# aleju/cat-generator

Hardware: AMD Instinct MI355X
Metric: images/sec per G+D step, G32up-c 32x32 RGB bs=128 per GPU (higher is better)
Workload: dtype f32

## Files before the change

### cat-generator_amd/csrc/common.h

```cpp
#pragma once
#include <hip/hip_runtime.h>
#include <algorithm>
#include <stdint.h>
#include <stdio.h>
#include <string.h>
#include "../../include/catgan.h"

namespace cg {

char* err_buf();
int fail(const char* fmt, ...);

inline hipStream_t S(void* s) { return reinterpret_cast<hipStream_t>(s); }

#define CG_HIP(call)                                                              \
    do {                                                                          \
        hipError_t e__ = (call);                                                  \
        if (e__ != hipSuccess)                                                    \
            return cg::fail("%s:%d %s -> %s", __FILE__, __LINE__, #call,          \
                            hipGetErrorString(e__));                              \
    } while (0)

#define CG_LAUNCH_CHECK()                                                         \
    do {                                                                          \
        hipError_t e__ = hipGetLastError();                                       \
        if (e__ != hipSuccess)                                                    \
            return cg::fail("%s:%d kernel launch -> %s", __FILE__, __LINE__,      \
                            hipGetErrorString(e__));                              \
    } while (0)

#define CG_REQUIRE(cond, ...)                                                     \
    do {                                                                          \
        if (!(cond)) return cg::fail(__VA_ARGS__);                                \
    } while (0)

constexpr int kNumCU = 256;

#ifndef CG_TIMING_PROBE
#define CG_TIMING_PROBE 0
#endif
#define CG_PROBE_HALF(fam, T) (((CG_TIMING_PROBE) & (fam)) ? ((T) + 1) / 2 : (T))
constexpr int kEwWgsPerCU = 4, kColReduceWgsPerCU = 1;

enum Opt {
    OPT_SKINNY, OPT_GEMM_BK32, OPT_WINO_BK, OPT_NN_TILE, OPT_TN_TILE, OPT_NN_SPLITS, OPT_TN_SPLITS,
    OPT_XCD_SWIZZLE, OPT_NN_GLDS, OPT_TN_GLDS, OPT_WINO_GLDS, OPT_PAD_SKIP, OPT_WINO3, OPT_COUNT
};
long opt(Opt o);

static inline int cdiv(long a, long b) { return (int)((a + b - 1) / b); }

constexpr size_t kColScratchBytes = 8u << 20;
void* col_scratch(hipStream_t stream);
hipStream_t queue_stream(hipStream_t ref, int cls, int slot);
int queue_class(hipStream_t ref, hipStream_t s);
void wgrad_discard_all();

constexpr int kSkinnyWgradBlocks = 512;
bool skinny_ok(int ngroups, int Cin, int Cout, int kH, int kW, int padH, int padW, int ups);
size_t skinny_wgrad_ws_bytes(int Cin, int Cout);
void skinny_valu_forward(hipStream_t st, const float* x, const float* w, const float* bias, float* y, int N, int H, int W, int Cin, int Cout);
void skinny_valu_wgrad(hipStream_t st, const float* x, const float* dy, float* part, float* bias_part, int N, int H, int W, int Cin, int Cout,
                       int blocks, long ppb);
bool skinny_mfma_ok(int Cin, int Cout, int H, int W);
int skinny_mfma_forward(hipStream_t st, const float* x, const float* w, const float* bias, float* y, int N, int H, int W, int Cin, int Cout);
int skinny_mfma_wgrad(hipStream_t st, const float* x, const float* dy, float* part, float* bias_part, int N, int H, int W, int Cin, int Cout,
                      int max_blocks);

bool head_wgrad_ok(int N, int T, int C, int Co);
int head_wgrad(hipStream_t st, const float* x, const float* dy, float* gw, float* gb, int N, int T, int C, int Co, float scale);
bool wino3_geom_ok(int ngroups, int N, int H, int W, int Cin, int Cout, int kH, int kW, int padH, int padW, int ups);
int wino3_note_pack(hipStream_t st, int n, const float* const* w, float* const* wf, float* const* wb, const int* Cout, const int* Cin,
                    const int* kH, const int* kW, const int* wb_map);
int wino3_forward(hipStream_t st, int ngroups, const float* const* x, const float* const* wpk, const float* const* bias, float* const* y,
                  int N, int H, int W);

static inline int ew_grid(long n, int per_block = 256) {
    long b = (n + per_block - 1) / per_block;
    if (b < 1) b = 1;
    const long cap = (long)kNumCU * kEwWgsPerCU;
    if (b > cap) b = cap;
    return (int)b;
}

__device__ __forceinline__ float u01(uint64_t seed, uint64_t ctr) {
    uint64_t z = seed + (ctr + 1) * 0x9E3779B97F4A7C15ull;
    z = (z ^ (z >> 30)) * 0xBF58476D1CE4E5B9ull;
    z = (z ^ (z >> 27)) * 0x94D049BB133111EBull;
    z = z ^ (z >> 31);
    return (float)(z >> 40) * (1.0f / 16777216.0f);
}
__device__ __forceinline__ float wave_sum(float v) {
#pragma unroll
    for (int off = 32; off > 0; off >>= 1) v += __shfl_down(v, off, 64);
    return v;
}
__device__ __forceinline__ double wave_sum(double v) {
#pragma unroll
    for (int off = 32; off > 0; off >>= 1) v += __shfl_down(v, off, 64);
    return v;
}

#ifndef CG_COL_HANDOVER
#define CG_COL_HANDOVER 3
#endif
__device__ __forceinline__ void st_agent(double* p, double v) {
#if CG_COL_HANDOVER == 4
    const unsigned long long old = __hip_atomic_exchange((unsigned long long*)p, (unsigned long long)__double_as_longlong(v),
                                                         __ATOMIC_RELAXED, __HIP_MEMORY_SCOPE_AGENT);
// ... 98 lines not shown
```

### cat-generator_amd/csrc/gemm.hip

```cpp
#include "common.h"
#include <stdlib.h>
#include <algorithm>
#include <mutex>
#include <type_traits>
#include <unordered_map>
#include <vector>

namespace {

typedef float f32x16 __attribute__((ext_vector_type(16)));
typedef unsigned int u32x4 __attribute__((ext_vector_type(4)));

constexpr int BK = 16;
constexpr unsigned OOB = 0x80000000u;
#ifdef CG_TRACE
__device__ unsigned long long* g_trace;
#define CG_STAMP(slot)                                                                                                  \
    do {                                                                                                                \
        if (threadIdx.x == 0 && g_trace) {                                                                              \
            const long wg = blockIdx.x + (long)gridDim.x * (blockIdx.y + (long)gridDim.y * blockIdx.z);                  \
            g_trace[wg * 8 + (slot)] = wall_clock64();                                                                  \
            if ((slot) == 0) {                                                                                          \
                g_trace[wg * 8 + 4] = __builtin_amdgcn_s_getreg((31 << 11) | 4);                       \
                g_trace[wg * 8 + 5] = __builtin_amdgcn_s_getreg((31 << 11) | 20);                     \
// ... 2189 lines not shown
    Geom g;
    if (check_dims(N, Hp, Wp, Cin, Cout, k, k, pad, pad, 1)) return 1;
    if (geom_phase_dgrad(g, N, Hp, Wp, Cin, Cout, k, pad)) return 1;
    return run_nn(cg::S(stream), g, 1, &dy, &wb_ph, nullptr, &dx_lo, ws, ws_bytes, "cg_conv2d_dgrad_ups2");
}

static size_t wgrad_ws_bytes_groups(int ngroups, int maxg, int N, int Hp, int Wp, int Cin, int Cout, int kH, int kW, int padH, int padW, int ups) {
    Geom g;
    if (ngroups < 1 || ngroups > maxg || conv_geom(g, N, Hp, Wp, Cin, Cout, kH, kW, padH, padW, ups)) return 0;
    const size_t reg = tn_ws_bytes(g, plan_tn(g, ngroups), ngroups);
    return cg::skinny_ok(ngroups, Cin, Cout, kH, kW, padH, padW, ups) ? std::max(reg, cg::skinny_wgrad_ws_bytes(Cin, Cout)) : reg;
}
size_t cg_conv2d_wgrad_workspace_bytes_grouped(int ngroups, int N, int Hp, int Wp, int Cin, int Cout, int kH, int kW,
                                               int padH, int padW, int ups) {
    return wgrad_ws_bytes_groups(ngroups, MAXG, N, Hp, Wp, Cin, Cout, kH, kW, padH, padW, ups);
}
size_t cg_conv2d_wgrad_workspace_bytes_strided(int ngroups, int N, int Hp, int Wp, int Cin, int Cout, int kH, int kW,
                                               int padH, int padW, int ups) {
    return wgrad_ws_bytes_groups(ngroups, kMaxStridedGroups, N, Hp, Wp, Cin, Cout, kH, kW, padH, padW, ups);
}
size_t cg_conv2d_wgrad_workspace_bytes(int N, int Hp, int Wp, int Cin, int Cout, int kH, int kW, int padH, int padW,
                                       int ups) {
    return cg_conv2d_wgrad_workspace_bytes_grouped(1, N, Hp, Wp, Cin, Cout, kH, kW, padH, padW, ups);
}

namespace {
std::mutex g_red_mu;
std::unordered_map<hipStream_t, std::vector<RedJob>> g_red_queue;

long red_cap() { return 0x7fffffffL; }

int small_reduce(hipStream_t st, bool defer, const RedJob& job, int ngroups) {
    if (defer) {
        std::lock_guard<std::mutex> lk(g_red_mu);
        g_red_queue[st].push_back(job);
        g_red_queue[st].back().block0 = ngroups;
        return 0;
    }
    const int nblocks = job.wblocks + job.bblocks;
    const long cap = std::max<long>(1, red_cap() / std::max(1, ngroups));
    dim3 sgrid((unsigned)std::min<long>(nblocks, cap), ngroups);
    if (job.ups)
        hipLaunchKernelGGL(wgrad_reduce_small_kernel<true>, sgrid, dim3(256), 0, st, job.part, job.bias_part, job.rp, job.Cin, job.Cout,
                           job.k, job.KK, job.pad, job.kp, job.S, job.P, job.scale, job.sstride, job.gstride, job.bsstride, job.wblocks, nblocks, 0);
    else
        hipLaunchKernelGGL(wgrad_reduce_small_kernel<false>, sgrid, dim3(256), 0, st, job.part, job.bias_part, job.rp, job.Cin, job.Cout,
                           job.k, job.KK, job.pad, job.kp, job.S, job.P, job.scale, job.sstride, job.gstride, job.bsstride, job.wblocks, nblocks, job.v4);
    CG_LAUNCH_CHECK();
    return 0;
}

int wgrad_impl(void* stream, int ngroups, const float* const* x, const float* const* dy, float* const* gw, float* const* gb, int N,
               int Hp, int Wp, int Cin, int Cout, int kH, int kW, int padH, int padW, int ups, float scale, void* ws, size_t ws_bytes,
               bool defer, long xgs = 0, long dgs = 0, long gws = 0, bool gemm_only = false);
}

int cg_conv2d_wgrad_grouped(void* stream, int ngroups, const float* const* x, const float* const* dy, float* const* gw,
                            float* const* gb, int N, int Hp, int Wp, int Cin, int Cout, int kH, int kW, int padH, int padW,
                            int ups, float scale, void* ws, size_t ws_bytes) {
    return wgrad_impl(stream, ngroups, x, dy, gw, gb, N, Hp, Wp, Cin, Cout, kH, kW, padH, padW, ups, scale, ws, ws_bytes, false);
}

int cg_conv2d_wgrad_grouped_deferred(void* stream, int ngroups, const float* const* x, const float* const* dy, float* const* gw,
                                     float* const* gb, int N, int Hp, int Wp, int Cin, int Cout, int kH, int kW, int padH, int padW,
                                     int ups, float scale, void* ws, size_t ws_bytes) {
    return wgrad_impl(stream, ngroups, x, dy, gw, gb, N, Hp, Wp, Cin, Cout, kH, kW, padH, padW, ups, scale, ws, ws_bytes, true);
}

int cg_conv2d_wgrad_strided(void* stream, int ngroups, const float* x, long x_stride, const float* dy, long dy_stride, float* gw,
                            long gw_stride, int N, int Hp, int Wp, int Cin, int Cout, int kH, int kW, int padH, int padW, int ups,
                            float scale, void* ws, size_t ws_bytes) {
    CG_REQUIRE(x && dy && gw && x_stride > 0 && dy_stride > 0 && gw_stride > 0, "cg_conv2d_wgrad_strided: bad arguments");
    CG_REQUIRE(ngroups >= 1 && ngroups <= kMaxStridedGroups, "cg_conv2d_wgrad_strided: 1..%d groups per launch", kMaxStridedGroups);
    return wgrad_impl(stream, ngroups, &x, &dy, &gw, nullptr, N, Hp, Wp, Cin, Cout, kH, kW, padH, padW, ups, scale, ws, ws_bytes, false,
                      x_stride, dy_stride, gw_stride);
}

int cg_conv2d_wgrad_gemm(void* stream, const float* x, const float* dy, int N, int Hp, int Wp, int Cin, int Cout, int kH, int kW, int padH,
                         int padW, int ups, void* ws, size_t ws_bytes) {
    CG_REQUIRE(x && dy && ws, "cg_conv2d_wgrad_gemm: null pointer");
    CG_REQUIRE(!cg::skinny_ok(1, Cin, Cout, kH, kW, padH, padW, ups), "cg_conv2d_wgrad_gemm: this geometry runs the skinny kernel, not the GEMM");
    float* gw = (float*)ws;
    return wgrad_impl(stream, 1, &x, &dy, &gw, nullptr, N, Hp, Wp, Cin, Cout, kH, kW, padH, padW, ups, 1.f, ws, ws_bytes, false, 0, 0, 0, true);
}

int cg_conv2d_wgrad_pending(void* stream, int* njobs) {
    CG_REQUIRE(njobs, "cg_conv2d_wgrad_pending: null pointer");
    std::lock_guard<std::mutex> lk(g_red_mu);
    auto it = g_red_queue.find(cg::S(stream));
    *njobs = it == g_red_queue.end() ? 0 : (int)it->second.size();
    return 0;
}

int cg_conv2d_wgrad_flush(void* stream) {
    hipStream_t st = cg::S(stream);
    std::vector<RedJob> jobs;
    {
        std::lock_guard<std::mutex> lk(g_red_mu);
        auto it = g_red_queue.find(st);
        if (it == g_red_queue.end() || it->second.empty()) return 0;
        jobs.swap(it->second);
    }
    for (size_t j0 = 0; j0 < jobs.size(); j0 += kRedJobs) {
        RedJobTable t;
        memset(&t, 0, sizeof(t));
        t.n = (int)std::min<size_t>(kRedJobs, jobs.size() - j0);
        int blocks = 0;
        for (int q = 0; q < t.n; ++q) {
            t.j[q] = jobs[j0 + q];
            const int ngroups = t.j[q].block0;
            t.j[q].block0 = blocks;
            blocks += ngroups * (t.j[q].wblocks + t.j[q].bblocks);
        }
        const int wgs = (int)std::min<long>(blocks, red_cap());
        hipLaunchKernelGGL(wgrad_reduce_batch_kernel, dim3(wgs), dim3(256), 0, st, t, blocks);
        CG_LAUNCH_CHECK();
    }
    return 0;
}

namespace {
int wgrad_impl(void* stream, int ngroups, const float* const* x, const float* const* dy, float* const* gw, float* const* gb, int N,
               int Hp, int Wp, int Cin, int Cout, int kH, int kW, int padH, int padW, int ups, float scale, void* ws, size_t ws_bytes,
               bool defer, long xgs, long dgs, long gws_, bool gemm_only) {
    CG_REQUIRE(x && dy && gw, "cg_conv2d_wgrad: null pointer");
    const bool strided = xgs != 0;
    CG_REQUIRE(ngroups >= 1 && ngroups <= (strided ? kMaxStridedGroups : MAXG), "cg_conv2d_wgrad: 1..%d groups per launch", strided ? kMaxStridedGroups : MAXG);
    CG_REQUIRE(!strided || (!gb && !defer), "cg_conv2d_wgrad: strided groups carry no bias gradient and are not deferred");
    TNArgs a;
    memset(&a, 0, sizeof(a));
    if (conv_geom(a.g, N, Hp, Wp, Cin, Cout, kH, kW, padH, padW, ups)) return 1;
    const Geom& g = a.g;
    if (!strided && cg::skinny_ok(ngroups, Cin, Cout, kH, kW, padH, padW, ups) && x[0] && dy[0] && gw[0] && (uintptr_t)x[0] % 16 == 0 && ws &&
        ws_bytes >= cg::skinny_wgrad_ws_bytes(Cin, Cout) && (long)N * Hp * Wp < 0x7fffffffL) {
        hipStream_t st = cg::S(stream);
        const long npix = (long)N * Hp * Wp;
        const long ppb = (npix + cg::kSkinnyWgradBlocks - 1) / cg::kSkinnyWgradBlocks;
        int blocks = (int)((npix + ppb - 1) / ppb);
        float* part = (float*)ws;
        float* bpart = part + (size_t)cg::kSkinnyWgradBlocks * 9 * Cin * Cout;
        float* gb0 = gb ? gb[0] : nullptr;
        if (cg::opt(cg::OPT_SKINNY) == 1 && cg::skinny_mfma_ok(Cin, Cout, Hp, Wp)) {
            blocks = cg::skinny_mfma_wgrad(st, x[0], dy[0], part, gb0 ? bpart : nullptr, N, Hp, Wp, Cin, Cout, cg::kSkinnyWgradBlocks / 2);
            if (blocks < 0) return 1;
        }
        else cg::skinny_valu_wgrad(st, x[0], dy[0], part, gb0 ? bpart : nullptr, N, Hp, Wp, Cin, Cout, blocks, ppb);
        CG_LAUNCH_CHECK();
        RedJob job;
        memset(&job, 0, sizeof(job));
        job.part = part; job.bias_part = bpart;
        job.rp.gw0 = gw[0]; job.rp.gb0 = gb0;
        job.Cin = Cin; job.Cout = Cout; job.k = 3; job.KK = 9; job.pad = 1; job.S = blocks; job.P = 1; job.scale = scale;
        job.sstride = 9L * Cin * Cout; job.gstride = 0; job.bsstride = Cout;
        job.wblocks = cg::cdiv(9L * Cin * Cout, 32); job.bblocks = gb0 ? cg::cdiv(Cout, 32) : 0;
        return small_reduce(st, defer, job, 1);
    }
    if (!strided && !gemm_only && ngroups == 1 && !ups && kH == Hp && kW == Wp && padH == 0 && padW == 0 && cg::opt(cg::OPT_PAD_SKIP) > 0 &&
        cg::opt(cg::OPT_TN_GLDS) && cg::head_wgrad_ok(N, kH * kW, Cin, Cout) && x[0] && dy[0] && gw[0] && (uintptr_t)x[0] % 16 == 0 &&
        (uintptr_t)dy[0] % 16 == 0 && (uintptr_t)gw[0] % 4 == 0)
        return cg::head_wgrad(cg::S(stream), x[0], dy[0], gw[0], gb ? gb[0] : nullptr, N, kH * kW, Cin, Cout, scale) != 0;
    TNPlan p = plan_tn(g, ngroups);
    const size_t need = tn_ws_bytes(g, p, ngroups);
    CG_REQUIRE(ws && ws_bytes >= need, "cg_conv2d_wgrad: workspace too small (%zu < %zu)", ws_bytes, need);
    const int nptr = strided ? 1 : ngroups;
    bool veca = Cin % 4 == 0, vecb = Cout % 4 == 0, any_gb = false;
    for (int i = 0; i < nptr; ++i) {
        CG_REQUIRE(x[i] && dy[i] && gw[i], "cg_conv2d_wgrad: null pointer (group %d)", i);
        veca = veca && ((uintptr_t)x[i] % 16 == 0);
        vecb = vecb && ((uintptr_t)dy[i] % 16 == 0);
        any_gb = any_gb || (gb && gb[i]);
    }
    if (strided) { veca = veca && xgs % 4 == 0; vecb = vecb && dgs % 4 == 0; }
    if (p.pm && !(veca && vecb)) p = plan_tn(g, ngroups, false);
    a.xgs = xgs; a.dgs = dgs;
    set4(a.x0, a.x1, a.x2, a.x3, x, nptr);
    set4(a.d0, a.d1, a.d2, a.d3, dy, nptr);
    a.ngroups = ngroups; a.part = (float*)ws; a.pchunk = p.pchunk;
    a.xcd_swizzle = (int)cg::opt(cg::OPT_XCD_SWIZZLE);
    const int ZP = ngroups * g.nphase;
    const long wplane = (long)g.Ktot * g.Cout;
    a.bias_part = any_gb ? (float*)ws + (size_t)p.splits * ZP * wplane : nullptr;
    hipStream_t st = cg::S(stream);
    dim3 grid(cg::cdiv(g.Ktot, p.tc.bm) * cg::cdiv(g.Cout, p.tc.bn), p.splits, ZP);
    if (p.pm && veca && vecb) a.pm_n = g.M / (g.Hg * g.Wg);
    if (a.pm_n || tng_ok(g, p.pchunk, veca, vecb)) {
        if (p.tc.bm == 128 && p.tc.bn == 128) launch_tng<128, 128, 2, 2>(a, grid, st);
        else if (p.tc.bm == 64 && p.tc.bn == 128) launch_tng<64, 128, 2, 2>(a, grid, st);
        else if (p.tc.bm == 128 && p.tc.bn == 64) launch_tng<128, 64, 2, 2>(a, grid, st);
        else if (p.tc.bm == 64 && p.tc.bn == 64) launch_tng<64, 64, 2, 2>(a, grid, st);
        else launch_tng<128, 32, 4, 1>(a, grid, st);
    }
    else if (p.tc.bm == 128 && p.tc.bn == 128) launch_tn<128, 128, 2, 2>(a, grid, st, veca, vecb);
    else if (p.tc.bm == 64 && p.tc.bn == 128) launch_tn<64, 128, 2, 2>(a, grid, st, veca, vecb);
    else if (p.tc.bm == 128 && p.tc.bn == 64) launch_tn<128, 64, 2, 2>(a, grid, st, veca, vecb);
    else if (p.tc.bm == 64 && p.tc.bn == 64) launch_tn<64, 64, 2, 2>(a, grid, st, veca, vecb);
    else launch_tn<128, 32, 4, 1>(a, grid, st, veca, vecb);
    CG_LAUNCH_CHECK();
    if (gemm_only) return 0;
    const int KK = kH * kW;
    int ci_t = KK == 1 ? 64 : 8;
    while (ci_t > 1 && (size_t)KK * ci_t * 33 * sizeof(float) > 60000) ci_t >>= 1;
    const size_t shb = (size_t)KK * ci_t * 33 * sizeof(float);
    dim3 rgrid(cg::cdiv(Cin, ci_t), cg::cdiv(Cout, 32));
    const long relems = (long)KK * Cin * Cout;
    const long sstride = (long)ZP * wplane;
    const int kp = ups ? phase_kp(kH, padH) : 0;
    if (strided && KK == 1 && !ups && !any_gb && Cin % 32 == 0 && Cout % 32 == 0 && g.nphase == 1) {
        hipLaunchKernelGGL(wgrad_reduce_t_kernel, dim3(Cin / 32, Cout / 32, ngroups), dim3(256), 0, st, (const float*)ws, gw[0], gws_, Cin, Cout,
                           p.splits, sstride, (long)g.nphase * wplane, scale);
        CG_LAUNCH_CHECK();
        return 0;
    }
    if ((long)rgrid.x * rgrid.y < cg::kNumCU) {
        RedJob job;
        memset(&job, 0, sizeof(job));
        job.rp.gws = strided ? gws_ : 0;
        set4(job.rp.gw0, job.rp.gw1, job.rp.gw2, job.rp.gw3, gw, nptr);
        set4(job.rp.gb0, job.rp.gb1, job.rp.gb2, job.rp.gb3, gb, nptr);
        job.part = (const float*)ws; job.bias_part = a.bias_part;
        job.Cin = Cin; job.Cout = Cout; job.k = kH; job.KK = KK; job.pad = padH; job.kp = ups ? kp : 0; job.S = p.splits; job.P = g.nphase;
        job.ups = ups ? 1 : 0; job.scale = scale;
        job.sstride = sstride; job.gstride = (long)g.nphase * wplane; job.bsstride = (long)ZP * Cout;
        job.wblocks = cg::cdiv(relems, 32); job.bblocks = any_gb ? cg::cdiv(Cout, 32) : 0;
        if (defer && KK == 1 && !ups && Cin % 32 == 0 && Cout % 32 == 0 && g.nphase == 1) {
            job.tr = 1; job.wblocks = (Cin / 32) * (Cout / 32);
        } else if (!ups && Cout % 4 == 0 && (uintptr_t)ws % 16 == 0 && sstride % 4 == 0 && job.gstride % 4 == 0) {
            job.v4 = 1; job.wblocks = cg::cdiv(relems, 128);
        }
        return small_reduce(st, defer, job, ngroups);
    }
    for (int gi = 0; gi < ngroups; ++gi) {
        const float* pg = (const float*)ws + (long)gi * g.nphase * wplane;
        float* gwi = strided ? gw[0] + (long)gi * gws_ : gw[gi];
        if (ups)
            hipLaunchKernelGGL(wgrad_reduce_kernel<true>, rgrid, dim3(256), shb, st, pg, gwi, Cin, Cout, kH, KK, padH, kp,
                               p.splits, scale, ci_t, sstride);
        else
            hipLaunchKernelGGL(wgrad_reduce_kernel<false>, rgrid, dim3(256), shb, st, pg, gwi, Cin, Cout, kH, KK, padH,
                               0, p.splits, scale, ci_t, sstride);
        CG_LAUNCH_CHECK();
        if (gb && gb[gi]) {
            hipLaunchKernelGGL(bias_part_reduce_kernel, dim3(cg::cdiv(Cout, 32)), dim3(256), 0, st,
                               (const float*)a.bias_part + (long)gi * g.nphase * Cout, gb[gi], p.splits, g.nphase,
                               (long)ZP * Cout, Cout, scale);
            CG_LAUNCH_CHECK();
        }
    }
    return 0;
}

}
// ... 37 lines not shown
    for (int i0 = 0; i0 < n; i0 += kPackBatch) {
        PackBatch b;
        memset(&b, 0, sizeof(b));
        b.n = std::min(kPackBatch, n - i0);
        int blocks = 0;
        for (int e = 0; e < b.n; ++e) {
            const int i = i0 + e;
            CG_REQUIRE(w_canonical[i] && (wf[i] || wb[i]) && Cout[i] > 0 && Cin[i] > 0 && kH[i] > 0 && kW[i] > 0,
                       "cg_pack_conv_weight_batch: bad layer %d", i);
            b.w[e] = w_canonical[i]; b.wf[e] = wf[i]; b.wb[e] = wb[i];
            b.Cout[e] = Cout[i]; b.Cin[e] = Cin[i]; b.KK[e] = kH[i] * kW[i];
            if (wb_map && wb_map[i]) b.map_mask |= 1ull << e;
            b.first[e] = blocks;
            blocks += cg::cdiv(Cin[i], 32) * cg::cdiv(Cout[i], 32) * b.KK[e];
        }
        b.first[b.n] = blocks;
        hipLaunchKernelGGL(pack_weight_batch_kernel, dim3(blocks), dim3(256), 0, cg::S(stream), b);
        CG_LAUNCH_CHECK();
    }
    return cg::wino3_note_pack(cg::S(stream), n, w_canonical, wf, wb, Cout, Cin, kH, kW, wb_map);
}

size_t cg_pack_conv_weight_ups2_floats(int Cout, int Cin, int k, int pad) {
    if (Cout <= 0 || Cin <= 0 || k <= 0 || (k & 1) == 0 || pad != (k - 1) / 2) return 0;
    const int kp = phase_kp(k, pad);
    return (size_t)4 * kp * kp * Cin * Cout;
}

int cg_pack_conv_weight_ups2(void* stream, const float* w, float* wf_ph, float* wb_ph, int Cout, int Cin, int k, int pad) {
    CG_REQUIRE(w && (wf_ph || wb_ph), "cg_pack_conv_weight_ups2: null pointer");
    CG_REQUIRE(Cout > 0 && Cin > 0 && k > 0 && (k & 1) == 1 && pad == (k - 1) / 2,
               "cg_pack_conv_weight_ups2: needs an odd kernel with pad=(k-1)/2");
    const int kp = phase_kp(k, pad);
    CG_REQUIRE(k * k <= 448, "cg_pack_conv_weight_ups2: kernel too large (%d taps)", k * k);
    const dim3 fgrid(cg::cdiv(Cin, 32), cg::cdiv(Cout, 32));
    if (k == 3 || k == 5) {
        if (k == 3)
            hipLaunchKernelGGL(pack_weight_ups2_fast_kernel<3>, fgrid, dim3(256), 0, cg::S(stream), w, wf_ph, wb_ph, Cout, Cin);
        else
            hipLaunchKernelGGL(pack_weight_ups2_fast_kernel<5>, fgrid, dim3(256), 0, cg::S(stream), w, wf_ph, wb_ph, Cout, Cin);
        CG_LAUNCH_CHECK();
        return 0;
    }
    const int ci_t = pack_ci_tile(Cin, k * k);
    hipLaunchKernelGGL(pack_weight_ups2_kernel, dim3(cg::cdiv(Cin, ci_t), cg::cdiv(Cout, 32)), dim3(256),
                       (size_t)32 * (ci_t * k * k + 1) * sizeof(float), cg::S(stream), w, wf_ph, wb_ph, Cout, Cin, k, pad, kp,
                       ci_t);
    CG_LAUNCH_CHECK();
    return 0;
}

}

void cg::wgrad_discard_all() {
    std::lock_guard<std::mutex> lk(g_red_mu);
    for (auto& kv : g_red_queue) kv.second.clear();
}
```

### cat-generator_amd/csrc/ops.hip

```cpp
#include "common.h"
#include <stdarg.h>
#include <stdlib.h>
#include <algorithm>

namespace cg {
char* err_buf() {
    static thread_local char buf[512] = {0};
    return buf;
}
int fail(const char* fmt, ...) {
    va_list ap;
    va_start(ap, fmt);
    vsnprintf(err_buf(), 512, fmt, ap);
    va_end(ap);
    return 1;
}

namespace {
struct OptDef { const char* name; long dflt; };
const OptDef kOptDefs[OPT_COUNT] = {
    {"CG_SKINNY", 1}, {"CG_GEMM_BK32", 1}, {"CG_WINO_BK", 0}, {"CG_NN_TILE", 0}, {"CG_TN_TILE", 0}, {"CG_NN_SPLITS", 0}, {"CG_TN_SPLITS", 0},
    {"CG_XCD_SWIZZLE", 7}, {"CG_NN_GLDS", 1}, {"CG_TN_GLDS", 1}, {"CG_WINO_GLDS", 1}, {"CG_PAD_SKIP", 20}, {"CG_WINO3", 1},
};
long g_opt_val[OPT_COUNT];
int g_opt_state[OPT_COUNT];
}

}
#include <chrono>
#include <mutex>
#include <unordered_map>
#include <vector>
namespace cg {
void* col_scratch(hipStream_t stream) {
    constexpr int kPool = 8, kReserve = 4;
    static std::unordered_map<hipStream_t, void*> blocks;
    static std::vector<void*> pool;
    static std::mutex mu;
    std::lock_guard<std::mutex> lk(mu);
    auto it = blocks.find(stream);
    if (it != blocks.end()) return it->second;
    hipStreamCaptureStatus st = hipStreamCaptureStatusNone;
    const bool capturing = stream && hipStreamIsCapturing(stream, &st) == hipSuccess && st != hipStreamCaptureStatusNone;
    if (capturing && pool.empty()) {
        cg::fail("column reduce: no scratch block left for a stream first used inside a graph capture (run one pass on it before cg_graph_begin)");
        return nullptr;
    }
    if (!capturing && (int)pool.size() <= kReserve) {
        char* p = nullptr;
        hipStreamCaptureMode mode = hipStreamCaptureModeRelaxed;
        (void)hipThreadExchangeStreamCaptureMode(&mode);
        const bool ok = hipMalloc((void**)&p, kColScratchBytes * kPool) == hipSuccess &&
                        hipMemsetAsync(p, 0, kColScratchBytes * kPool, stream) == hipSuccess &&
                        hipStreamSynchronize(stream) == hipSuccess;
        (void)hipThreadExchangeStreamCaptureMode(&mode);
        if (!ok) {
            (void)hipGetLastError();
            if (pool.empty()) { cg::fail("column reduce: cannot allocate %zu bytes of scratch", kColScratchBytes * kPool); return nullptr; }
        } else
            for (int i = kPool - 1; i >= 0; --i) pool.insert(pool.begin(), p + (size_t)i * kColScratchBytes);
    }
    void* blk = pool.back();
    pool.pop_back();
    blocks[stream] = blk;
    return blk;
}
namespace {
__global__ void queue_probe_spin_k(unsigned long long ticks, int* sink) {
    const unsigned long long t0 = wall_clock64();
    while (wall_clock64() - t0 < ticks) { }
    if (ticks == ~0ull) *sink = 1;
}
struct QueuePool {
    std::vector<hipStream_t> s;
    std::unordered_map<hipStream_t, std::vector<int>> cls;
// ... 1892 lines not shown
```

### cat-generator_amd/csrc/winograd.hip

```cpp
#include "common.h"
#include <algorithm>
#include <type_traits>
#include <stdlib.h>

namespace {

typedef float f32x16 __attribute__((ext_vector_type(16)));

__device__ __forceinline__ float4 ld4(const float* p) { return *reinterpret_cast<const float4*>(p); }
__device__ __forceinline__ float wf4c(const float4& v, int i) { return i == 0 ? v.x : (i == 1 ? v.y : (i == 2 ? v.z : v.w)); }
__device__ __forceinline__ float4 f4add(float4 a, float4 b) { return make_float4(a.x + b.x, a.y + b.y, a.z + b.z, a.w + b.w); }
__device__ __forceinline__ float4 f4sub(float4 a, float4 b) { return make_float4(a.x - b.x, a.y - b.y, a.z - b.z, a.w - b.w); }

template <int MODE>
__global__ __launch_bounds__(256) void wino_input_transform_kernel(const float* __restrict__ src, float* __restrict__ V,
                                                                   int N, int Hl, int Wl, int C, int Cs) {
    const int cq_n = C >> 2;
    const int tH = Hl >> 1, tW = Wl >> 1;
    const long T = (long)N * tH * tW;
    const long total = T * cq_n;
    for (long idx = blockIdx.x * 256L + threadIdx.x; idx < total; idx += gridDim.x * 256L) {
        const int cq = (int)(idx % cq_n);
        const long tile = idx / cq_n;
        const int tj = (int)(tile % tW);
// ... 615 lines not shown
        }
    sh[rl][cl] = a;
    __syncthreads();
    if (rl == 0 && co < Cout) {
        double t = 0.0;
#pragma unroll
        for (int r = 0; r < 8; ++r) t += sh[r][cl];
        gb[co] += scale * (float)t;
    }
}

__device__ __host__ __forceinline__ int wino_phase_map(int a, int d) { return ((a + d - 2) >> 1) - ((a - 2) >> 1); }

__global__ __launch_bounds__(256) void wino_wgrad_finish_kernel(const float* __restrict__ dUt, float* __restrict__ gw, int Cout,
                                                                int Cin, float scale) {
    const long total = (long)Cout * Cin;
    const long xs = 4L * Cout * Cin;
    for (long idx = blockIdx.x * 256L + threadIdx.x; idx < total; idx += gridDim.x * 256L) {
        const int ci = (int)(idx % Cin);
        const int co = (int)(idx / Cin);
        float acc[25];
#pragma unroll
        for (int t = 0; t < 25; ++t) acc[t] = 0.f;
#pragma unroll
        for (int p = 0; p < 4; ++p) {
            float u[4][4];
#pragma unroll
            for (int xi = 0; xi < 16; ++xi) u[xi >> 2][xi & 3] = dUt[xi * xs + ((long)p * Cout + co) * Cin + ci];
            float t[3][4];
#pragma unroll
            for (int c = 0; c < 4; ++c) {
                t[0][c] = u[0][c] + 0.5f * (u[1][c] + u[2][c]);
                t[1][c] = 0.5f * (u[1][c] - u[2][c]);
                t[2][c] = 0.5f * (u[1][c] + u[2][c]) + u[3][c];
            }
            float g[3][3];
#pragma unroll
            for (int r = 0; r < 3; ++r) {
                g[r][0] = t[r][0] + 0.5f * (t[r][1] + t[r][2]);
                g[r][1] = 0.5f * (t[r][1] - t[r][2]);
                g[r][2] = 0.5f * (t[r][1] + t[r][2]) + t[r][3];
            }
#pragma unroll
            for (int dy = 0; dy < 5; ++dy)
#pragma unroll
                for (int dx = 0; dx < 5; ++dx) acc[dy * 5 + dx] += g[wino_phase_map(p >> 1, dy)][wino_phase_map(p & 1, dx)];
        }
        float* dst = gw + idx * 25;
#pragma unroll
        for (int t = 0; t < 25; ++t) dst[t] += scale * acc[t];
    }
}


__device__ __host__ __forceinline__ int wino22_phase_map(int a, int d) { return ((a + d - 1) >> 1) - ((a - 1) >> 1); }


static bool wino_dims_ok(int N, int Hp, int Wp, int Cin, int Cout) {
    return N > 0 && Hp > 0 && Wp > 0 && (Hp & 1) == 0 && (Wp & 1) == 0 && Cin > 0 && Cout > 0 && Cin % 128 == 0 &&
           Cout % 128 == 0  && (long)N * Hp * Wp * std::max(Cin, 4 * Cout) * 4L < (1L << 40);
}

}

extern "C" {

size_t cg_conv2d_ups2_wino_supported(int N, int Hp, int Wp, int Cin, int Cout, int k, int pad) {
    return k == 5 && pad == 2 && wino_dims_ok(N, Hp, Wp, Cin, Cout) ? 1 : 0;
}
size_t cg_conv2d_ups2_wino_v_floats(int N, int Hp, int Wp, int C) {
    return (size_t)16 * ((size_t)N * (Hp / 2) * (Wp / 2)) * C;
}
size_t cg_conv2d_ups2_wino_u_floats(int Cin, int Cout) { return (size_t)4 * 16 * Cin * Cout; }

int cg_conv2d_ups2_wino_pack(void* stream, const float* wf_ph, const float* wb_ph, float* u_fwd, float* u_bwd, int Cout,
                             int Cin) {
    CG_REQUIRE((wf_ph && u_fwd) || (wb_ph && u_bwd), "cg_conv2d_ups2_wino_pack: null pointer");
    CG_REQUIRE(Cin % 4 == 0 && Cout % 4 == 0, "cg_conv2d_ups2_wino_pack: channel counts must be multiples of 4");
    if (wf_ph && u_fwd) {
        const long total = 4L * Cin * (Cout / 4);
        hipLaunchKernelGGL(wino_filter_transform_kernel<false>, dim3(cg::ew_grid(total)), dim3(256), 0, cg::S(stream), wf_ph,
                           u_fwd, Cin, Cout);
        CG_LAUNCH_CHECK();
    }
    if (wb_ph && u_bwd) {
        const long total = 4L * Cout * (Cin / 4);
        hipLaunchKernelGGL(wino_filter_transform_kernel<true>, dim3(cg::ew_grid(total)), dim3(256), 0, cg::S(stream), wb_ph,
                           u_bwd, Cout, Cin);
        CG_LAUNCH_CHECK();
    }
    return 0;
}

static int wino_gemm_launch(void* stream, const float* v, const float* u, const float* bias, float* y, int N, int Hp, int Wp,
                            int Cin, int Cout, int dgrad, float* stats, int npos = 16, int kslices = 1);

int cg_conv2d_ups2_wino_gemm(void* stream, const float* v, const float* u, const float* bias, float* y, int N, int Hp, int Wp,
                             int Cin, int Cout, int dgrad) {
    return wino_gemm_launch(stream, v, u, bias, y, N, Hp, Wp, Cin, Cout, dgrad, nullptr);
}

size_t cg_conv2d_ups2_wino_stats_rows(int N, int Hp, int Wp, int Cin, int Cout) {
    if (!wino_dims_ok(N, Hp, Wp, Cin, Cout)) return 0;
    return (size_t)4 * cg::cdiv((long)N * (Hp / 2) * (Wp / 2), 64) * 2;
}

// ... 159 lines not shown
}
size_t cg_conv2d_ups2_wino_dgrad_part_floats(int N, int Hp, int Wp, int Cin, int Cout) {
    const int sl = wino_dgrad_slices(N, Hp, Wp, Cin, Cout);
    return sl > 1 ? (size_t)sl * N * Hp * Wp * Cin : 0;
}
int cg_conv2d_ups2_wino_dgrad_split(void* stream, const float* dy, const float* u_bwd, float* dx_lo, float* v_dy, float* part, int N, int Hp,
                                    int Wp, int Cin, int Cout) {
    const int sl = wino_dgrad_slices(N, Hp, Wp, Cin, Cout);
    if (sl <= 1 || !part) return cg_conv2d_ups2_wino_dgrad(stream, dy, u_bwd, dx_lo, v_dy, N, Hp, Wp, Cin, Cout);
    CG_REQUIRE(dy && u_bwd && dx_lo && v_dy, "cg_conv2d_ups2_wino_dgrad_split: null pointer");
    const int T = N * (Hp / 2) * (Wp / 2);
    hipLaunchKernelGGL(wino_input_transform_kernel<1>, dim3(cg::ew_grid((long)T * Cout)), dim3(256), 0, cg::S(stream), dy, v_dy, N, Hp, Wp, 4 * Cout, Cout);
    CG_LAUNCH_CHECK();
    if (wino_gemm_launch(stream, v_dy, u_bwd, nullptr, part, N, Hp, Wp, Cin, Cout, 1, nullptr, 16, sl)) return 1;
    const long n = (long)T * 4 * Cin;
    if (sl == 4) hipLaunchKernelGGL(wino22_sum_kernel<4>, dim3(cg::ew_grid(n / 4)), dim3(256), 0, cg::S(stream), part, dx_lo, n / 4, n);
    else hipLaunchKernelGGL(wino22_sum_kernel<2>, dim3(cg::ew_grid(n / 4)), dim3(256), 0, cg::S(stream), part, dx_lo, n / 4, n);
    CG_LAUNCH_CHECK();
    return 0;
}

static size_t wino_align(size_t b) { return (b + 255) / 256 * 256; }

size_t cg_conv2d_ups2_wino_wgrad_workspace_bytes(int N, int Hp, int Wp, int Cin, int Cout) {
    if (!wino_dims_ok(N, Hp, Wp, Cin, Cout)) return 0;
    const size_t T = (size_t)N * (Hp / 2) * (Wp / 2);
    return wino_align(16 * T * 4 * Cout * sizeof(float)) + wino_align((size_t)16 * 4 * Cout * Cin * sizeof(float)) +
           wino_align(std::max(sizeof(double) * Cout, (size_t)cg::kNumCU * 8 * 4 * Cout * sizeof(float))) +

           cg_conv2d_wgrad_workspace_bytes_strided(16, (int)T, 1, 1, Cin, 4 * Cout, 1, 1, 0, 0, 0);
}

int cg_conv2d_ups2_wino_wgrad(void* stream, const float* v, const float* dy, float* gw_canonical, float* gb, int N, int Hp,
                              int Wp, int Cin, int Cout, float scale, void* ws, size_t ws_bytes) {
    CG_REQUIRE(v && dy && gw_canonical, "cg_conv2d_ups2_wino_wgrad: null pointer");
    CG_REQUIRE(wino_dims_ok(N, Hp, Wp, Cin, Cout), "cg_conv2d_ups2_wino_wgrad: unsupported dimensions");
    const size_t need = cg_conv2d_ups2_wino_wgrad_workspace_bytes(N, Hp, Wp, Cin, Cout);
    CG_REQUIRE(ws && ws_bytes >= need && (uintptr_t)ws % 16 == 0, "cg_conv2d_ups2_wino_wgrad: workspace too small (%zu < %zu)",
               ws_bytes, need);
    hipStream_t st = cg::S(stream);
    const int T = N * (Hp / 2) * (Wp / 2);
    const int C4 = 4 * Cout;
    char* base = (char*)ws;
    float* mdy = (float*)base;                    base += wino_align((size_t)16 * T * C4 * sizeof(float));
    float* dut = (float*)base;                    base += wino_align((size_t)16 * C4 * Cin * sizeof(float));
    const size_t bws_bytes = wino_align(std::max(sizeof(double) * Cout, (size_t)cg::kNumCU * 8 * 4 * Cout * sizeof(float)));
    void* bws = base;                             base += bws_bytes;
    void* tws = base;
    const size_t tws_bytes = ws_bytes - (size_t)(base - (char*)ws);
    const bool fuse = false;
    const int tgrid = (int)cg::ew_grid((long)T * Cout);
    hipLaunchKernelGGL(wino_dy_transform_kernel, dim3(tgrid), dim3(256), 0, st, dy, mdy, N, Hp, Wp, Cout, fuse ? (float*)bws : nullptr);
    CG_LAUNCH_CHECK();
    CG_HIP(hipMemsetAsync(dut, 0, (size_t)16 * C4 * Cin * sizeof(float), st));
    const int groups_per_launch = 16;
    for (int q = 0; q < 16; q += groups_per_launch) {
        if (cg_conv2d_wgrad_strided(stream, groups_per_launch, v + q * (long)T * Cin, (long)T * Cin, mdy + q * (long)T * C4, (long)T * C4,
                                    dut + q * (long)C4 * Cin, (long)C4 * Cin, T, 1, 1, Cin, C4, 1, 1, 0, 0, 0, 1.f, tws, tws_bytes)) return 1;
    }
    hipLaunchKernelGGL(wino_wgrad_finish_kernel, dim3(cg::ew_grid((long)Cout * Cin)), dim3(256), 0, st, dut, gw_canonical, Cout,
                       Cin, scale);
    CG_LAUNCH_CHECK();
    if (fuse) {
        hipLaunchKernelGGL(wino_bias_finish_kernel, dim3(cg::cdiv(Cout, 32)), dim3(256), 0, st, (const float*)bws, tgrid, Cout, gb, scale);
        CG_LAUNCH_CHECK();
        return 0;
    }
    if (gb) return cg_bias_grad(stream, dy, gb, (long)N * 4 * Hp * Wp, Cout, scale, bws, wino_align(sizeof(double) * Cout));
    return 0;
}



}
```

Baseline: 22840.

## Fuse split-K partial reduction into Winograd wgrad inverse-transform finish kernel

Winograd weight-gradient GEMMs now run in gemm-only mode and hand back their split-K partial buffers. A new finish kernel sums the splits, applies the inverse Winograd transform and accumulates into the canonical 5x5 weights in one pass. This removes the memset of the transformed-gradient buffer, the separate split reduction, and a round trip through that buffer. The cost is a more involved finish kernel that re-reads all partial splits and depends on the GEMM's internal partial layout.

Measured after the change: 22750. About the same (-0.4%).

```diff
diff --git a/cat-generator_amd/csrc/common.h b/cat-generator_amd/csrc/common.h
--- a/cat-generator_amd/csrc/common.h
+++ b/cat-generator_amd/csrc/common.h
@@ -44,7 +44,7 @@
 
 enum Opt {
     OPT_SKINNY, OPT_GEMM_BK32, OPT_WINO_BK, OPT_NN_TILE, OPT_TN_TILE, OPT_NN_SPLITS, OPT_TN_SPLITS,
-    OPT_XCD_SWIZZLE, OPT_NN_GLDS, OPT_TN_GLDS, OPT_WINO_GLDS, OPT_PAD_SKIP, OPT_WINO3, OPT_COUNT
+    OPT_XCD_SWIZZLE, OPT_NN_GLDS, OPT_TN_GLDS, OPT_WINO_GLDS, OPT_PAD_SKIP, OPT_WINO3, OPT_WINO_WGRAD_FUSED, OPT_COUNT
 };
 long opt(Opt o);
 
@@ -55,6 +55,9 @@
 hipStream_t queue_stream(hipStream_t ref, int cls, int slot);
 int queue_class(hipStream_t ref, hipStream_t s);
 void wgrad_discard_all();
+struct WgradPartials { const float* part; int splits, rows, cols; long split_stride, group_stride; };
+int wgrad_strided_gemm(void* stream, int ngroups, const float* x, long x_stride, const float* dy, long dy_stride, int N, int Hp, int Wp,
+                       int Cin, int Cout, int kH, int kW, int padH, int padW, int ups, void* ws, size_t ws_bytes, WgradPartials* left);
 
 constexpr int kSkinnyWgradBlocks = 512;
 bool skinny_ok(int ngroups, int Cin, int Cout, int kH, int kW, int padH, int padW, int ups);
diff --git a/cat-generator_amd/csrc/gemm.hip b/cat-generator_amd/csrc/gemm.hip
--- a/cat-generator_amd/csrc/gemm.hip
+++ b/cat-generator_amd/csrc/gemm.hip
@@ -2265,7 +2265,7 @@
 
 int wgrad_impl(void* stream, int ngroups, const float* const* x, const float* const* dy, float* const* gw, float* const* gb, int N,
                int Hp, int Wp, int Cin, int Cout, int kH, int kW, int padH, int padW, int ups, float scale, void* ws, size_t ws_bytes,
-               bool defer, long xgs = 0, long dgs = 0, long gws = 0, bool gemm_only = false);
+               bool defer, long xgs = 0, long dgs = 0, long gws = 0, bool gemm_only = false, cg::WgradPartials* left = nullptr);
 }
 
 int cg_conv2d_wgrad_grouped(void* stream, int ngroups, const float* const* x, const float* const* dy, float* const* gw,
@@ -2335,7 +2335,7 @@
 namespace {
 int wgrad_impl(void* stream, int ngroups, const float* const* x, const float* const* dy, float* const* gw, float* const* gb, int N,
                int Hp, int Wp, int Cin, int Cout, int kH, int kW, int padH, int padW, int ups, float scale, void* ws, size_t ws_bytes,
-               bool defer, long xgs, long dgs, long gws_, bool gemm_only) {
+               bool defer, long xgs, long dgs, long gws_, bool gemm_only, cg::WgradPartials* left) {
     CG_REQUIRE(x && dy && gw, "cg_conv2d_wgrad: null pointer");
     const bool strided = xgs != 0;
     CG_REQUIRE(ngroups >= 1 && ngroups <= (strided ? kMaxStridedGroups : MAXG), "cg_conv2d_wgrad: 1..%d groups per launch", strided ? kMaxStridedGroups : MAXG);
@@ -2409,7 +2409,13 @@
     else if (p.tc.bm == 64 && p.tc.bn == 64) launch_tn<64, 64, 2, 2>(a, grid, st, veca, vecb);
     else launch_tn<128, 32, 4, 1>(a, grid, st, veca, vecb);
     CG_LAUNCH_CHECK();
-    if (gemm_only) return 0;
+    if (gemm_only) {
+        if (left) {
+            left->part = (const float*)ws; left->splits = p.splits; left->rows = g.Ktot; left->cols = g.Cout;
+            left->split_stride = (long)ZP * wplane; left->group_stride = (long)g.nphase * wplane;
+        }
+        return 0;
+    }
     const int KK = kH * kW;
     int ci_t = KK == 1 ? 64 : 8;
     while (ci_t > 1 && (size_t)KK * ci_t * 33 * sizeof(float) > 60000) ci_t >>= 1;
@@ -2553,6 +2559,15 @@
 
 }
 
+int cg::wgrad_strided_gemm(void* stream, int ngroups, const float* x, long x_stride, const float* dy, long dy_stride, int N, int Hp, int Wp,
+                           int Cin, int Cout, int kH, int kW, int padH, int padW, int ups, void* ws, size_t ws_bytes, WgradPartials* left) {
+    CG_REQUIRE(x && dy && ws && left && x_stride > 0 && dy_stride > 0, "wgrad_strided_gemm: bad arguments");
+    CG_REQUIRE(ngroups >= 1 && ngroups <= kMaxStridedGroups, "wgrad_strided_gemm: 1..%d groups per launch", kMaxStridedGroups);
+    float* gw = (float*)ws;
+    return wgrad_impl(stream, ngroups, &x, &dy, &gw, nullptr, N, Hp, Wp, Cin, Cout, kH, kW, padH, padW, ups, 1.f, ws, ws_bytes, false,
+                      x_stride, dy_stride, 1, true, left);
+}
+
 void cg::wgrad_discard_all() {
     std::lock_guard<std::mutex> lk(g_red_mu);
     for (auto& kv : g_red_queue) kv.second.clear();
diff --git a/cat-generator_amd/csrc/ops.hip b/cat-generator_amd/csrc/ops.hip
--- a/cat-generator_amd/csrc/ops.hip
+++ b/cat-generator_amd/csrc/ops.hip
@@ -21,6 +21,7 @@
 const OptDef kOptDefs[OPT_COUNT] = {
     {"CG_SKINNY", 1}, {"CG_GEMM_BK32", 1}, {"CG_WINO_BK", 0}, {"CG_NN_TILE", 0}, {"CG_TN_TILE", 0}, {"CG_NN_SPLITS", 0}, {"CG_TN_SPLITS", 0},
     {"CG_XCD_SWIZZLE", 7}, {"CG_NN_GLDS", 1}, {"CG_TN_GLDS", 1}, {"CG_WINO_GLDS", 1}, {"CG_PAD_SKIP", 20}, {"CG_WINO3", 1},
+    {"CG_WINO_WGRAD_FUSED", 1},
 };
 long g_opt_val[OPT_COUNT];
 int g_opt_state[OPT_COUNT];
diff --git a/cat-generator_amd/csrc/winograd.hip b/cat-generator_amd/csrc/winograd.hip
--- a/cat-generator_amd/csrc/winograd.hip
+++ b/cat-generator_amd/csrc/winograd.hip
@@ -691,6 +691,86 @@
     }
 }
 
+constexpr int kWfCo = 32, kWfCi = 4;
+constexpr int kWfRow = 40;
+__device__ __forceinline__ float4 wino_split_sum(const float* __restrict__ src, int S, long sstride) {
+    float4 s = make_float4(0.f, 0.f, 0.f, 0.f);
+    int sp = 0;
+    for (; sp + 4 <= S; sp += 4) {
+        const float4 p0 = ld4(src + (long)sp * sstride), p1 = ld4(src + (long)(sp + 1) * sstride);
+        const float4 p2 = ld4(src + (long)(sp + 2) * sstride), p3 = ld4(src + (long)(sp + 3) * sstride);
+        s = f4add(f4add(f4add(f4add(s, p0), p1), p2), p3);
+    }
+    for (; sp < S; ++sp) s = f4add(s, ld4(src + (long)sp * sstride));
+    return s;
+}
+__global__ __launch_bounds__(256) void wino_wgrad_finish_fused_kernel(cg::WgradPartials P, float* __restrict__ gw, int Cout, int Cin,
+                                                                      float scale, int vec) {
+    __shared__ __attribute__((aligned(16))) float su[64 * kWfCi * kWfRow];
+    __shared__ __attribute__((aligned(16))) float sg[kWfCo * kWfCi * 25];
+    const int tid = threadIdx.x;
+    const int nci = Cin / kWfCi;
+    const int ci0 = ((int)blockIdx.x % nci) * kWfCi, co0 = ((int)blockIdx.x / nci) * kWfCo;
+    {
+        const int c4 = tid & 7, ci = (tid >> 3) & 3;
+#pragma unroll
+        for (int j = 0; j < 8; ++j) {
+            const int q = (tid >> 5) + 8 * j, p = q >> 4, xi = q & 15;
+            const float* src = P.part + xi * P.group_stride + (long)(ci0 + ci) * P.cols + p * Cout + co0 + 4 * c4;
+            *reinterpret_cast<float4*>(&su[(q * kWfCi + ci) * kWfRow + 4 * c4]) = wino_split_sum(src, P.splits, P.split_stride);
+        }
+    }
+    __syncthreads();
+    if (tid < kWfCo * kWfCi) {
+        const int ci = tid & 3, co = tid >> 2;
+        float acc[25];
+#pragma unroll
+        for (int t = 0; t < 25; ++t) acc[t] = 0.f;
+#pragma unroll
+        for (int p = 0; p < 4; ++p) {
+            float u[4][4];
+#pragma unroll
+            for (int xi = 0; xi < 16; ++xi) u[xi >> 2][xi & 3] = su[((p * 16 + xi) * kWfCi + ci) * kWfRow + co];
+            float t[3][4];
+#pragma unroll
+            for (int c = 0; c < 4; ++c) {
+                t[0][c] = u[0][c] + 0.5f * (u[1][c] + u[2][c]);
+                t[1][c] = 0.5f * (u[1][c] - u[2][c]);
+                t[2][c] = 0.5f * (u[1][c] + u[2][c]) + u[3][c];
+            }
+            float g[3][3];
+#pragma unroll
+            for (int r = 0; r < 3; ++r) {
+                g[r][0] = t[r][0] + 0.5f * (t[r][1] + t[r][2]);
+                g[r][1] = 0.5f * (t[r][1] - t[r][2]);
+                g[r][2] = 0.5f * (t[r][1] + t[r][2]) + t[r][3];
+            }
+#pragma unroll
+            for (int dy = 0; dy < 5; ++dy)
+#pragma unroll
+                for (int dx = 0; dx < 5; ++dx) acc[dy * 5 + dx] += g[wino_phase_map(p >> 1, dy)][wino_phase_map(p & 1, dx)];
+        }
+#pragma unroll
+        for (int t = 0; t < 25; ++t) sg[tid * 25 + t] = acc[t];
+    }
+    __syncthreads();
+    if (vec) {
+        for (int i = tid; i < kWfCo * kWfCi * 25 / 4; i += 256) {
+            const int r = i / 25, q = i - r * 25;
+            float* dst = gw + ((long)(co0 + r) * Cin + ci0) * 25 + 4 * q;
+            const float4 a = *reinterpret_cast<const float4*>(&sg[r * (kWfCi * 25) + 4 * q]);
+            float4 g = *reinterpret_cast<const float4*>(dst);
+            g.x += scale * a.x; g.y += scale * a.y; g.z += scale * a.z; g.w += scale * a.w;
+            *reinterpret_cast<float4*>(dst) = g;
+        }
+    } else {
+        for (int i = tid; i < kWfCo * kWfCi * 25; i += 256) {
+            const int r = i / (kWfCi * 25), q = i - r * (kWfCi * 25);
+            gw[((long)(co0 + r) * Cin + ci0) * 25 + q] += scale * sg[i];
+        }
+    }
+}
+
 
 __device__ __host__ __forceinline__ int wino22_phase_map(int a, int d) { return ((a + d - 1) >> 1) - ((a - 1) >> 1); }
 
@@ -956,15 +1036,22 @@
     const int tgrid = (int)cg::ew_grid((long)T * Cout);
     hipLaunchKernelGGL(wino_dy_transform_kernel, dim3(tgrid), dim3(256), 0, st, dy, mdy, N, Hp, Wp, Cout, fuse ? (float*)bws : nullptr);
     CG_LAUNCH_CHECK();
-    CG_HIP(hipMemsetAsync(dut, 0, (size_t)16 * C4 * Cin * sizeof(float), st));
-    const int groups_per_launch = 16;
-    for (int q = 0; q < 16; q += groups_per_launch) {
-        if (cg_conv2d_wgrad_strided(stream, groups_per_launch, v + q * (long)T * Cin, (long)T * Cin, mdy + q * (long)T * C4, (long)T * C4,
-                                    dut + q * (long)C4 * Cin, (long)C4 * Cin, T, 1, 1, Cin, C4, 1, 1, 0, 0, 0, 1.f, tws, tws_bytes)) return 1;
-    }
-    hipLaunchKernelGGL(wino_wgrad_finish_kernel, dim3(cg::ew_grid((long)Cout * Cin)), dim3(256), 0, st, dut, gw_canonical, Cout,
-                       Cin, scale);
-    CG_LAUNCH_CHECK();
+    if (cg::opt(cg::OPT_WINO_WGRAD_FUSED) != 0) {
+        cg::WgradPartials left;
+        if (cg::wgrad_strided_gemm(stream, 16, v, (long)T * Cin, mdy, (long)T * C4, T, 1, 1, Cin, C4, 1, 1, 0, 0, 0, tws, tws_bytes, &left)) return 1;
+        CG_REQUIRE(left.rows == Cin && left.cols == C4 && (uintptr_t)left.part % 16 == 0 && left.split_stride % 4 == 0 && left.group_stride % 4 == 0,
+                   "cg_conv2d_ups2_wino_wgrad: unexpected partial layout");
+        static_assert(128 % kWfCo == 0 && 128 % kWfCi == 0, "wino_dims_ok: planes are multiples of 128");
+        hipLaunchKernelGGL(wino_wgrad_finish_fused_kernel, dim3((Cout / kWfCo) * (Cin / kWfCi)), dim3(256), 0, st, left, gw_canonical, Cout, Cin,
+                           scale, (uintptr_t)gw_canonical % 16 == 0 ? 1 : 0);
+        CG_LAUNCH_CHECK();
+    } else {
+        CG_HIP(hipMemsetAsync(dut, 0, (size_t)16 * C4 * Cin * sizeof(float), st));
+        if (cg_conv2d_wgrad_strided(stream, 16, v, (long)T * Cin, mdy, (long)T * C4, dut, (long)C4 * Cin, T, 1, 1, Cin, C4, 1, 1, 0, 0, 0, 1.f, tws,
+                                    tws_bytes)) return 1;
+        hipLaunchKernelGGL(wino_wgrad_finish_kernel, dim3(cg::ew_grid((long)Cout * Cin)), dim3(256), 0, st, dut, gw_canonical, Cout, Cin, scale);
+        CG_LAUNCH_CHECK();
+    }
     if (fuse) {
         hipLaunchKernelGGL(wino_bias_finish_kernel, dim3(cg::cdiv(Cout, 32)), dim3(256), 0, st, (const float*)bws, tgrid, Cout, gb, scale);
         CG_LAUNCH_CHECK();
```
